# fallenshock/SinDDM

Measured on AMD Instinct MI355X. Metric: diffusion steps/sec (finest scale) + imgs/sec full multi-scale sample, 1/2/4/8 GPU, higher is better.
Workload: dtype f32 (3x3 convs: binary16 hi/lo split products -- Winograd-domain GEMMs with all 4 MFMA terms, fp32 accumulate; fp32-equivalent, error vs float64 = the fp32 oracle's: tests/test_gpu_h2.py; everything else fp32); 1 GPU; C3: 6-scale pyramid, T=1000, finest scale 411x512, batch 64 per GPU, dim=160; batch_per_gpu=64, global_batch=64, scale=5, parallelism=independent chains over 1 GPU(s), one all-gather of the images

## Files before the change

### include/sinddm_hip_debug.h

```cpp
#ifndef SINDDM_HIP_DEBUG_H
#define SINDDM_HIP_DEBUG_H

#include <stddef.h>
#include <stdint.h>

#ifdef __cplusplus
extern "C" {
#endif

int sinddm_prof_begin(void);
int sinddm_prof_end(double* conv_ms_total, int64_t* conv_launches, double* conv_flops_total);
int sinddm_prof_end2(double* conv_ms_total, int64_t* conv_launches, double* conv_flops_total,
                     double* conv_exec_flops_total);
int sinddm_prof_end3(int kind, double* ms_total, int64_t* launches, double* flops_total,
                     double* exec_flops_total, int reset);

int sinddm_debug_conv_path(int dim, int B, int H, int W);

int sinddm_debug_infer_path(int dim, int B, int H, int W);

int sinddm_debug_head_path(int dim, int B, int H, int W);
int sinddm_debug_head_offsets(int dim, int64_t out[3]);
int sinddm_debug_head(const float* packed, const float* g, const float* x_in, float* eps_out, int dim, int B, int H, int W,
                      int Wp, void* stream);

int sinddm_debug_train_path(int dim, int B, int H, int W);

int sinddm_debug_block_train(const float* params, const float* packed, const float* packed_bwd, int dim, int l,
                             const float* x, const float* cond_bias, const float* grad_y, float* y, float* grad_x,
                             float* grad_params, float* dcond, int B, int H, int W, void* ws, size_t ws_bytes,
                             void* stream);

int sinddm_debug_wgrad_map(int Cin, int Cout, int64_t ntiles, int ncu, uint32_t* wg_out, int wg_cap, int32_t* splits_out,
                           int splits_cap);

#ifdef __cplusplus
}
#endif
#endif
```

### sinddm_amd/_lib.py

```python
from __future__ import annotations

import ctypes as C
import os
from typing import Optional

import torch

_HERE = os.path.dirname(os.path.abspath(__file__))
LIB_PATH = os.path.join(_HERE, "libsinddm_hip.so")

ABI_SYMBOLS = (
    "sinddm_abi_version", "sinddm_param_count", "sinddm_param_tensors", "sinddm_param_offset",
    "sinddm_packed_count", "sinddm_workspace_bytes", "sinddm_pack_weights", "sinddm_net_forward",
    "sinddm_q_sample", "sinddm_reverse_step", "sinddm_reverse_step_edit", "sinddm_upsample_bilinear", "sinddm_prof_begin", "sinddm_prof_end", "sinddm_prof_end2", "sinddm_prof_end3", "sinddm_debug_wgrad_map", "sinddm_debug_conv_path",
    "sinddm_debug_block_train", "sinddm_debug_infer_path", "sinddm_debug_train_path",
    "sinddm_train_workspace_bytes", "sinddm_packed_bwd_count", "sinddm_pack_weights_bwd",
    "sinddm_net_forward_train", "sinddm_net_backward", "sinddm_l1_loss_fwd_bwd", "sinddm_adam_ema_step",
    "sinddm_cond_embed", "sinddm_cond_stride", "sinddm_sample_chain", "sinddm_sample_chain2", "sinddm_sample_chain_ex",
    "sinddm_normal_fill", "sinddm_wrap_halo", "sinddm_upsample_bilinear_wrap", "sinddm_sample_chain_tile",
    "sinddm_sample_chain_keep", "sinddm_reverse_step_keep", "sinddm_normal_fill_samples", "sinddm_sample_chain_seeds",
    "sinddm_debug_head_path", "sinddm_debug_head_offsets", "sinddm_debug_head",
)


ABI_VERSION = 3
DIM_FP32_CONVS = 0x10000
TILE_HALO = 16


class StepCoefs(C.Structure):
    _fields_ = [("mode", C.c_int), ("clip", C.c_int),
                ("sqrt_recip_ac_t", C.c_float), ("sqrt_recipm1_ac_t", C.c_float),
                ("coef1_t", C.c_float), ("coef2_t", C.c_float),
                ("gamma_t", C.c_float), ("gamma_tm1", C.c_float),
                ("sqrt_ac_tm1", C.c_float), ("sqrt_ac_t", C.c_float), ("sqrt_1m_ac_t", C.c_float),
                ("sqrt_1m_ac_tm1_mvar", C.c_float), ("sigma", C.c_float)]


class ChainOpts(C.Structure):
    _fields_ = [("edit_w", C.c_void_p), ("edit_c", C.c_void_p), ("noise", C.c_void_p)]


class KeepOpts(C.Structure):
    _fields_ = [("mask", C.c_void_p), ("x0", C.c_void_p), ("ab", C.POINTER(C.c_float))]


class SinddmError(RuntimeError):
    pass


_lib: Optional[C.CDLL] = None


def load() -> C.CDLL:
    global _lib
    if _lib is not None:
        return _lib
    if not os.path.exists(LIB_PATH):
        raise SinddmError(
# ... 17 lines not shown
        "sinddm_workspace_bytes": (sz, [i, i, i, i]),
        "sinddm_pack_weights": (i, [p, p, i, p]),
        "sinddm_net_forward": (i, [p, p, p, p, i, f, p, i, i, i, i, p, sz, p]),
        "sinddm_cond_embed": (i, [p, p, i, f, i, i, p, p, p, p]),
        "sinddm_cond_stride": (i, [i]),
        "sinddm_q_sample": (i, [p, p, p, p, p, p, p, p, i, i, i64, p]),
        "sinddm_reverse_step": (i, [p, p, p, p, p, C.POINTER(StepCoefs), i64, p]),
        "sinddm_reverse_step_edit": (i, [p, p, p, p, p, C.POINTER(StepCoefs), p, p, i, i, i, p]),
        "sinddm_sample_chain": (i, chain[:-2] + [C.POINTER(C.c_int)]),
        "sinddm_sample_chain2": (i, chain),
        "sinddm_sample_chain_ex": (i, chain + [C.POINTER(ChainOpts)]),
        "sinddm_sample_chain_tile": (i, chain + [C.POINTER(ChainOpts), i, i]),
        "sinddm_sample_chain_keep": (i, chain + [C.POINTER(ChainOpts), i, i, C.POINTER(KeepOpts)]),
        "sinddm_sample_chain_seeds": (i, chain + [C.POINTER(ChainOpts), i, i, C.POINTER(KeepOpts), p]),
        "sinddm_normal_fill_samples": (i, [p, i, i64, p, C.c_uint64, p]),
        "sinddm_reverse_step_keep": (i, [p, p, p, p, p, C.POINTER(StepCoefs), p, p, p, p, f, f, i, i, i, p]),
        "sinddm_wrap_halo": (i, [p, p, i, i, i, i, i, p]),
        "sinddm_upsample_bilinear_wrap": (i, [p, p, i, i, i, i, i, i, i, p]),
        "sinddm_normal_fill": (i, [p, i64, C.c_uint64, C.c_uint64, p]),
        "sinddm_upsample_bilinear": (i, [p, p, i, i, i, i, i, p]),
        "sinddm_prof_begin": (i, []),
        "sinddm_prof_end": (i, [C.POINTER(C.c_double), C.POINTER(C.c_int64), C.POINTER(C.c_double)]),
        "sinddm_prof_end2": (i, [C.POINTER(C.c_double), C.POINTER(C.c_int64), C.POINTER(C.c_double),
                                 C.POINTER(C.c_double)]),
        "sinddm_prof_end3": (i, [i, C.POINTER(C.c_double), C.POINTER(C.c_int64), C.POINTER(C.c_double),
                                 C.POINTER(C.c_double), i]),
        "sinddm_debug_wgrad_map": (i, [i, i, i64, i, C.POINTER(C.c_uint32), i, C.POINTER(C.c_int32), i]),
        "sinddm_debug_conv_path": (i, [i, i, i, i]),
        "sinddm_debug_infer_path": (i, [i, i, i, i]),
        "sinddm_debug_train_path": (i, [i, i, i, i]),
        "sinddm_debug_head_path": (i, [i, i, i, i]),
        "sinddm_debug_head_offsets": (i, [i, C.POINTER(C.c_int64)]),
        "sinddm_debug_head": (i, [p, p, p, p, i, i, i, i, i, p]),
        "sinddm_debug_block_train": (i, [p, p, p, i, i, p, p, p, p, p, p, p, i, i, i, p, sz, p]),
        "sinddm_train_workspace_bytes": (sz, [i, i, i, i]),
        "sinddm_packed_bwd_count": (i64, [i]),
        "sinddm_pack_weights_bwd": (i, [p, p, i, p]),
        "sinddm_net_forward_train": (i, [p, p, p, p, i, f, p, i, i, i, i, p, sz, p]),
        "sinddm_net_backward": (i, [p, p, p, p, p, p, p, i, i, i, i, p, sz, p]),
        "sinddm_l1_loss_fwd_bwd": (i, [p, p, p, p, i64, f, p]),
        "sinddm_adam_ema_step": (i, [p, p, p, p, p, f, f, f, f, f, f, f, i, i64, p]),
    }
    for name, (res, args) in sig.items():
        if not hasattr(lib, name):
            continue
        fn = getattr(lib, name)
        fn.restype = res
        fn.argtypes = args
    _lib = lib
    return lib


def missing_symbols():
    lib = load()
    return [s for s in ABI_SYMBOLS if not hasattr(lib, s)]


def check(rc: int, what: str) -> None:
    if rc != 0:
        kind = {-1: "bad argument", -2: "unsupported shape", -3: "workspace too small"}.get(rc, f"hipError {rc}")
        raise SinddmError(f"{what} failed: {kind}")


def ptr(t: Optional[torch.Tensor]) -> Optional[int]:
    if t is None:
        return None
# ... 10 lines not shown
```

### sinddm_amd/csrc/head.h

```cpp
#pragma once
#include "common.h"

namespace sinddm {

#ifndef SINDDM_HEAD_COLLAPSE
#define SINDDM_HEAD_COLLAPSE 1
#endif

constexpr int HEAD_GROUP = 16;

struct HeadPackArgs {
    long long dst;
    long long c2_w, c2_b, res_w, res_b;
    long long fin_w, fin_b;
    int half, dim;
};
__global__ __launch_bounds__(256) void head_pack_kernel(const float* __restrict__ params, float* __restrict__ packed,
                                                        HeadPackArgs a) {
    const int nc = a.half * CHANNELS * 9, nr = a.dim * CHANNELS;
    const int i = blockIdx.x * 256 + threadIdx.x;
    if (i >= nc + nr + CHANNELS) return;
    const float* wf = params + a.fin_w;
    double s = 0.;
    if (i < nc) {
        const int tap = i % 9, o = (i / 9) % CHANNELS, ci = i / (9 * CHANNELS);
        for (int m = 0; m < a.half; ++m)
            s += (double)wf[o * a.half + m] * (double)params[a.c2_w + ((long long)m * a.half + ci) * 9 + tap];
    } else if (i < nc + nr) {
        const int j = i - nc, o = j % CHANNELS, ci = j / CHANNELS;
        for (int m = 0; m < a.half; ++m) s += (double)wf[o * a.half + m] * (double)params[a.res_w + (long long)m * a.dim + ci];
    } else {
        const int o = i - nc - nr;
        for (int m = 0; m < a.half; ++m)
            s += (double)wf[o * a.half + m] * ((double)params[a.c2_b + m] + (double)params[a.res_b + m]);
        s += (double)params[a.fin_b + o];
    }
    packed[a.dst + i] = (float)s;
}

inline int head_pack_launch(const NetPlan& P, const float* params, float* packed, hipStream_t st) {
    const BlockPlan& b = P.blk[3];
    HeadPackArgs a{};
    a.dst = P.pk_hc;
    a.c2_w = b.c2_w; a.c2_b = b.c2_b; a.res_w = b.res_w; a.res_b = b.res_b;
    a.fin_w = P.fin_w; a.fin_b = P.fin_b;
    a.half = P.half; a.dim = P.dim;
    const long long total = P.npacked - P.pk_hc;
    hipLaunchKernelGGL(head_pack_kernel, dim3((unsigned)((total + 255) / 256)), dim3(256), 0, st, params, packed, a);
    SINDDM_LAUNCH_CHECK();
    return 0;
}

struct HeadEps {
    const float* g;
    const float* xin;
    const float* wc;
    const float* wr;
    const float* bc;
    int half, dim, H, Wp;

    __device__ __forceinline__ void operator()(int b, int q, f32x4 (&e)[3]) const {
        const int qpr = Wp >> 2;
        const int y = q / qpr, x = (q - y * qpr) * 4;
        const int plane = H * Wp;
        constexpr int OOBI = 0x40000000;
        int oq[3], ol[3], orr[3];
#pragma unroll
        for (int r = 0; r < 3; ++r) {
            const int gy = y + r - 1;
            const bool ok = gy >= 0 && gy < H;
            const int base = (gy * Wp + x) * 4;
            oq[r] = ok ? base : OOBI;
            ol[r] = (ok && x >= 4) ? base - 4 : OOBI;
            orr[r] = (ok && x + 4 < Wp) ? base + 16 : OOBI;
        }
#pragma unroll
        for (int o = 0; o < 3; ++o) e[o] = f32x4{bc[o], bc[o], bc[o], bc[o]};
        const float* gb = g + (size_t)b * half * plane;
        auto fetch = [&](int c, float (&v)[3][6]) __attribute__((always_inline)) {
            const __amdgpu_buffer_rsrc_t rs =
                __builtin_amdgcn_make_buffer_rsrc(const_cast<float*>(gb + (size_t)c * plane), 0, plane * 4, 0x00020000);
#pragma unroll
            for (int r = 0; r < 3; ++r) {
                const f32x4 m = __builtin_bit_cast(f32x4, __builtin_amdgcn_raw_buffer_load_b128(rs, oq[r], 0, 0));
                v[r][0] = __builtin_bit_cast(float, __builtin_amdgcn_raw_buffer_load_b32(rs, ol[r], 0, 0));
                v[r][1] = m[0]; v[r][2] = m[1]; v[r][3] = m[2]; v[r][4] = m[3];
                v[r][5] = __builtin_bit_cast(float, __builtin_amdgcn_raw_buffer_load_b32(rs, orr[r], 0, 0));
            }
        };
        float in[3][6];
        fetch(0, in);
        f32x4 p[3] = {{0.f, 0.f, 0.f, 0.f}, {0.f, 0.f, 0.f, 0.f}, {0.f, 0.f, 0.f, 0.f}};
        for (int c = 0; c < half; ++c) {
            float nx[3][6];
            fetch(c + 1 < half ? c + 1 : c, nx);
            const float* wk = wc + c * 27;
#pragma unroll
            for (int r = 0; r < 3; ++r)
#pragma unroll
                for (int o = 0; o < 3; ++o)
#pragma unroll
                    for (int kx = 0; kx < 3; ++kx)
#pragma unroll
                        for (int j = 0; j < 4; ++j) p[o][j] = fmaf(wk[o * 9 + r * 3 + kx], in[r][j + kx], p[o][j]);
            if ((c + 1) % HEAD_GROUP == 0 || c + 1 == half) {
#pragma unroll
                for (int o = 0; o < 3; ++o) {
                    e[o] += p[o];
                    p[o] = f32x4{0.f, 0.f, 0.f, 0.f};
                }
            }
#pragma unroll
            for (int r = 0; r < 3; ++r)
#pragma unroll
                for (int k = 0; k < 6; ++k) in[r][k] = nx[r][k];
        }
        const float* xb = xin + (size_t)b * dim * plane + (size_t)q * 4;
        for (int c0 = 0; c0 < dim; c0 += HEAD_GROUP) {
            const int c1 = c0 + HEAD_GROUP < dim ? c0 + HEAD_GROUP : dim;
            f32x4 p[3] = {{0.f, 0.f, 0.f, 0.f}, {0.f, 0.f, 0.f, 0.f}, {0.f, 0.f, 0.f, 0.f}};
#pragma unroll 8
            for (int c = c0; c < c1; ++c) {
                const f32x4 v = *reinterpret_cast<const f32x4*>(xb + (size_t)c * plane);
#pragma unroll
                for (int o = 0; o < 3; ++o)
#pragma unroll
                    for (int j = 0; j < 4; ++j) p[o][j] = fmaf(wr[c * 3 + o], v[j], p[o][j]);
            }
#pragma unroll
            for (int o = 0; o < 3; ++o) e[o] += p[o];
        }
    }
};

struct FinalConvEps {
    const float* a;
    const float* w;
    const float* bias;
    int C;
    size_t plane;

    __device__ __forceinline__ void operator()(int b, int q, f32x4 (&e)[3]) const {
        const float* src = a + (size_t)b * C * plane + (size_t)q * 4;
#pragma unroll
        for (int o = 0; o < 3; ++o) e[o] = f32x4{bias[o], bias[o], bias[o], bias[o]};
#pragma unroll 8
        for (int c = 0; c < C; ++c) {
            const f32x4 v = *reinterpret_cast<const f32x4*>(src + (size_t)c * plane);
// ... 34 lines not shown
```

### sinddm_amd/csrc/internal.h

```cpp
#pragma once
#include "common.h"

namespace sinddm {

struct PackSeg {
    long long dst;
    long long count;
    long long w;
    long long w2;
    int kind;
    int cin, cout, taps, nch, mt, co_lds;
    int transpose;
};
struct PackArgs {
    PackSeg seg[32];
    int nseg;
    long long total;
};
int pack_launch(const float* params, float* packed, const PackArgs& a, hipStream_t st);

struct TrainBufs {
    float* cond;
    float* emb;
    float* hpre;
    float* cvec;
    float* mvec;
    float* h[4];
    float* u[4];
    float* g[4];
    float* o[4];
    float* s[4];
    float* dcond;
    float* small;
    float* wscr;
    float* amax;
};

struct ChainStep;
int net_forward_impl(const NetPlan& P, const float* params, const float* packed, const float* x, const int64_t* t_dev,
                     int t_host, float scale, float* out, int B, int H, int W, void* ws, size_t ws_bytes,
                     hipStream_t st, const TrainBufs* tb, const ChainStep* cs = nullptr);

int block_forward(const NetPlan& P, int l, const float* params, const float* packed, const float* cur, const float* cond,
                  int cond_stride, float* hbuf, float* gbuf, float* obuf, float* upre, int B, int H, int W, hipStream_t st,
                  int Wt = 0, float* amax = nullptr, bool skip2 = false);
int conv3x3_path(int cout, int cin, int coblks, int B, int H, int W);

struct ConvArgs;
bool wh_applies(const NetPlan& P, int B, int H, int W, int cin, int cout);
bool wh_enabled();
int wh_conv(const ConvArgs& c, hipStream_t st);
int wh_pack(const float* w, float* wsinv, void* img, int cin, int cout, int transpose, hipStream_t st);
int amax_tensor_launch(const float* x, float* amax, int B, long long per_sample, hipStream_t st);

int dwconv_launch(const float* x, const float* w, const float* bias, const float* cond, int cond_stride,
                  const float* addt, int flip, float* out, int B, int C, int H, int W, hipStream_t st, int pi = 0, int po = 0,
                  float* amax = nullptr);

}
```

### sinddm_amd/csrc/plan.h

```cpp
#pragma once
#include <stdint.h>

namespace sinddm {

constexpr int KC = 8;
constexpr int TIME_DIM = 32;
constexpr int CHANNELS = 3;

inline bool wh_plan_ok(int cin, int cout) { return cin >= 32 && cin % 16 == 0 && cout % 80 == 0; }
inline long long wh_plan_halfs(int cin, int cout) { return (long long)(cout / 80) * (cin / 16) * 24 * 5 * 512; }

struct BlockPlan {
    int cin, cout;
    int64_t mlp_w, mlp_b, tr_w, tr_b, dw_w, dw_b, c1_w, c1_b, c2_w, c2_b, res_w, res_b;
    int mt;
    int coblks;
    int co_lds;
    int nch1;
    int nch2;
    int nchr;
    int64_t pk_c1, pk_c2, pk_res, pk_b1, pk_b2;
    int nchw1, nchw2;
    int64_t pk_wc1, pk_wc2;
    int64_t pk_w1f, pk_w2f;
    int64_t pk_q1, pk_q2, pk_qs1, pk_qs2;
    int cond_off;
};

struct NetPlan {
    int dim, half;
    BlockPlan blk[4];
    int64_t tm0_w, tm0_b, tm2_w, tm2_b, fin_w, fin_b;
    int64_t nparams, npacked;
    int64_t pk_zero;
    int64_t pk_hc, pk_hr, pk_hb;
    int ntensors;
    int64_t tensor_off[64];
    int cond_stride;
    bool fp32_convs;
    bool ok;
};

inline int mt_for(int cout) { return (cout % 80 == 0) ? 5 : ((cout % 32 == 0) ? 2 : 1); }
inline int co_lds_for(int mt) { int m = mt * 16; return (m % 32 == 16) ? m : m + 16; }

inline NetPlan make_plan(int dim_arg) {
    NetPlan p{};
    const int dim = dim_arg & 0xFFFF;
    p.fp32_convs = (dim_arg & 0x10000) != 0;
    if (dim_arg < 0 || (dim_arg >> 17) != 0) { p.ok = false; return p; }
    p.ok = dim >= 2 && dim % 2 == 0 && dim <= 1024;
    p.dim = dim;
    p.half = dim / 2;
    int64_t o = 0;
    int nt = 0;
    auto take = [&](int64_t n) { int64_t r = o; p.tensor_off[nt++] = r; o += n; return r; };
    p.tm0_w = take(TIME_DIM * 4 * TIME_DIM * 2);
    p.tm0_b = take(TIME_DIM * 4);
    p.tm2_w = take(TIME_DIM * TIME_DIM * 4);
    p.tm2_b = take(TIME_DIM);
    const int cins[4] = {CHANNELS, p.half, dim, dim};
    const int couts[4] = {p.half, dim, dim, p.half};
    int64_t q = 0;
    int coff = 0;
    for (int l = 0; l < 4; ++l) {
        BlockPlan& b = p.blk[l];
        b.cin = cins[l];
        b.cout = couts[l];
        b.mlp_w = take(TIME_DIM * TIME_DIM);
        b.mlp_b = take(TIME_DIM);
        b.tr_w = take((int64_t)b.cin * TIME_DIM);
        b.tr_b = take(b.cin);
        b.dw_w = take((int64_t)b.cin * 25);
        b.dw_b = take(b.cin);
        b.c1_w = take((int64_t)b.cout * b.cin * 9);
        b.c1_b = take(b.cout);
        b.c2_w = take((int64_t)b.cout * b.cout * 9);
        b.c2_b = take(b.cout);
        if (b.cin != b.cout) {
            b.res_w = take((int64_t)b.cout * b.cin);
            b.res_b = take(b.cout);
        } else {
            b.res_w = b.res_b = -1;
// ... 47 lines not shown
```

### sinddm_amd/csrc/sinddm_fwd.hip

```cpp
#include "conv_mfma.h"
#include "conv_wino.h"
#include "conv_wino4.h"
#include "conv_wh.h"
#include "internal.h"
#include "step_tail.h"
#include <type_traits>
namespace sinddm {

ConvProfiler& conv_profiler() {
    static ConvProfiler p;
    return p;
}

__global__ void pack_kernel(const float* __restrict__ params, float* __restrict__ packed, PackArgs a) {
    long long i = (long long)blockIdx.x * blockDim.x + threadIdx.x;
    if (i >= a.total) return;
    int s = 0;
    long long base = 0;
    while (s < a.nseg - 1 && i >= base + a.seg[s].count) { base += a.seg[s].count; ++s; }
    const PackSeg& g = a.seg[s];
    const long long j = i - base;
    float v = 0.0f;
    if (g.kind == 0) {
        const int co_l = (int)(j % g.co_lds);
// ... 414 lines not shown
        const f32x4 qr = __builtin_bit_cast(f32x4, __builtin_amdgcn_raw_buffer_load_b128(rsx, (rowok && rok) ? base + 16 : OOBI, 0, 0));
        const float in[8] = {ql[2], ql[3], qm[0], qm[1], qm[2], qm[3], qr[0], qr[1]};
#pragma unroll
        for (int r = 0; r < DWR_ROWS; ++r) {
            const int ky = ir - r;
            if (ky >= 0 && ky < 5) {
#pragma unroll
                for (int kx = 0; kx < 5; ++kx) {
#pragma unroll
                    for (int cc = 0; cc < 4; ++cc) acc[r][cc] = fmaf(wk[ky * 5 + kx], in[cc + kx], acc[r][cc]);
                }
            }
        }
    }
    float mx = 0.f;
#pragma unroll
    for (int r = 0; r < DWR_ROWS; ++r) {
        const int gy = y0 + r;
        if (colok && gy < H) {
            const size_t o = plane + (size_t)gy * W + x4;
            f32x4 v = acc[r];
            if (addt) v += *reinterpret_cast<const f32x4*>(addt + o);
            if (x4 + 4 > Wt) {
#pragma unroll
                for (int cc = 0; cc < 4; ++cc) v[cc] = x4 + cc < Wt ? v[cc] : 0.0f;
            }
            mx = fmaxf(fmaxf(mx, fmaxf(fabsf(v[0]), fabsf(v[1]))), fmaxf(fabsf(v[2]), fabsf(v[3])));
            *reinterpret_cast<f32x4*>(out + o) = v;
        }
    }
    if (amax) amax_publish(mx, amax + (size_t)b * AMAX_STRIDE);
}

#ifndef SINDDM_DW_ROWS
#define SINDDM_DW_ROWS 1
#endif

int dwconv_launch(const float* x, const float* w, const float* bias, const float* cond, int cond_stride,
                  const float* addt, int flip, float* out, int B, int C, int H, int W, hipStream_t st, int pi, int po,
                  float* amax) {
    if (pi <= 0) pi = W;
    if (po <= 0) po = W;
    if (SINDDM_DW_ROWS && pi % 4 == 0 && po == pi && pi >= 192) {
        const int bandsX = (pi + 255) / 256, bandsY = (H + 4 * DWR_ROWS - 1) / (4 * DWR_ROWS);
        hipLaunchKernelGGL(dwconv5_rows_kernel, dim3(bandsX * bandsY, C, B), dim3(256), 0, st, x, w, bias, cond, cond_stride,
                           addt, flip, out, C, H, pi, bandsX, W, amax);
        SINDDM_LAUNCH_CHECK();
        return 0;
    }
    const int tilesX = (W + DW_TW - 1) / DW_TW, tilesY = (H + DW_TH - 1) / DW_TH;
    const int groupsX = (tilesX + DW_NX - 1) / DW_NX;
    hipLaunchKernelGGL(dwconv5_kernel, dim3(groupsX * tilesY, C, B), dim3(256), 0, st, x, w, bias, cond, cond_stride,
                       addt, flip, out, C, H, W, groupsX, pi, po, amax);
    SINDDM_LAUNCH_CHECK();
    return 0;
}

__global__ __launch_bounds__(256) void conv3x3_c3_gelu_kernel(const float* __restrict__ in, const float* __restrict__ w,
                                                              const float* __restrict__ bias, float* __restrict__ out,
                                                              float* __restrict__ out_pre, int H, int W, int Cout,
                                                              int co_per_block, int Wt, float* __restrict__ amax) {
    const int HW = H * W;
    const int b = blockIdx.y;
    const int co0 = blockIdx.z * co_per_block;
    const int co1 = min(Cout, co0 + co_per_block);
    const int p = blockIdx.x * 256 + threadIdx.x;
    const bool live = p < HW;
    const int pc = live ? p : HW - 1;
    const int y = pc / W, x = pc - y * W;
    const float* src = in + (size_t)b * 3 * HW;
    float v[27];
#pragma unroll
    for (int ci = 0; ci < 3; ++ci)
#pragma unroll
        for (int ky = 0; ky < 3; ++ky)
#pragma unroll
            for (int kx = 0; kx < 3; ++kx) {
                const int gy = y + ky - 1, gx = x + kx - 1;
                const bool ok = gy >= 0 && gy < H && gx >= 0 && gx < W;
                v[ci * 9 + ky * 3 + kx] = ok ? src[(size_t)ci * HW + (size_t)gy * W + gx] : 0.0f;
            }
    float* dst = out + (size_t)b * Cout * HW + pc;
    float* dpre = out_pre ? out_pre + (size_t)b * Cout * HW + pc : nullptr;
    f32x2 vp[13];
#pragma unroll
    for (int j = 0; j < 13; ++j) vp[j] = f32x2{v[2 * j], v[2 * j + 1]};
// ... 250 lines not shown
        if (b.cin != 3 && !(b.pk_wc1 >= 0 && b.cin % 4 == 0)) return false;
    }
    return true;
}
static int fwd_pitch(const NetPlan& P, int W) { return (W % 4 != 0 && plan_pads_rows(P)) ? (W + 3) / 4 * 4 : W; }
static size_t fwd_xpad_bytes(const NetPlan& P, int B, int H, int W) {
    return fwd_pitch(P, W) != W ? align_up((size_t)B * CHANNELS * H * fwd_pitch(P, W) * sizeof(float), 256) : 0;
}
static size_t fwd_workspace_core(const NetPlan& P, int B, int H, int W) {
    const size_t act = align_up((size_t)B * P.dim * H * fwd_pitch(P, W) * sizeof(float), 256);
    return cond_region_bytes(P, B) + 4 * act + fwd_xpad_bytes(P, B, H, W);
}
static size_t fwd_workspace_bytes(const NetPlan& P, int B, int H, int W) {
    return fwd_workspace_core(P, B, H, W) + 2 * cond_region_bytes(P, (B + 1) / 2) + 4096;
}

struct ChainStep {
    const float* cond_row;
    const float* x_tilde;
    float* x_next;
    TailArgs tail;
};

template <class F>
static void tail_dispatch(const TailArgs& t, F&& f) {
    auto keep = [&](auto e, auto n) { t.km ? f(e, n, std::true_type{}) : f(e, n, std::false_type{}); };
    auto noise = [&](auto e) { t.nz ? keep(e, std::true_type{}) : keep(e, std::false_type{}); };
    t.ew ? noise(std::true_type{}) : noise(std::false_type{});
}

static bool head_applies(const TrainBufs* tb, int H, int Wp) {
    return SINDDM_HEAD_COLLAPSE && !tb && Wp % 4 == 0 && (long long)H * Wp < (1LL << 28);
}
static HeadEps head_eps(const NetPlan& P, const float* packed, const float* g, const float* xin, int H, int Wp) {
    return HeadEps{g, xin, packed + P.pk_hc, packed + P.pk_hr, packed + P.pk_hb, P.half, P.dim, H, Wp};
}

int conv3x3_path(int cout, int cin, int coblks, int B, int H, int W) {
    if (!wino_enabled() || cout % 4 != 0) return 0;
    const bool f24 = mt_for(cout) == 5 && cout % 80 == 0 && cin >= 16 && cin % 16 == 0;
    const bool v3 = SINDDM_WINO_V3 && f24 &&
                    (long long)B * ((W + 31) / 32) * ((H + 3) / 4) * coblks >= SINDDM_V3_MIN_ITEMS_PER_CU * wino2_cu_count();
    if (v3 && SINDDM_WINO_V4 && conv_wino4_applies(B, H, W, coblks)) return 4;
    return v3 ? 3 : 2;
}

int block_forward(const NetPlan& P, int l, const float* params, const float* packed, const float* cur, const float* cond,
                  int cond_stride, float* hbuf, float* gbuf, float* obuf, float* upre, int B, int H, int W, hipStream_t st,
                  int Wt, float* amax, bool skip2) {
    const BlockPlan& b = P.blk[l];
    const bool wha = amax && b.pk_q1 >= 0 && conv_wh_applies(P.fp32_convs, B, H, W, b.cin, b.cout);
    const bool whb = !skip2 && amax && b.pk_q2 >= 0 && conv_wh_applies(P.fp32_convs, B, H, W, b.cout, b.cout);
    int rc = Wt > 0 ? dwconv_launch(cur, params + b.dw_w, params + b.dw_b, cond, cond_stride, nullptr, 0, hbuf, B, b.cin, H,
                                    Wt, st, W, W, wha ? amax : nullptr)
                    : dwconv_launch(cur, params + b.dw_w, params + b.dw_b, cond, cond_stride, nullptr, 0, hbuf, B, b.cin, H,
                                    W, st, 0, 0, wha ? amax : nullptr);
    if (rc) return rc;
    const bool wino = wino_enabled();
    ConvArgs c1{};
    c1.in = hbuf; c1.bias = packed + b.pk_b1; c1.out = gbuf;
    c1.B = B; c1.H = H; c1.W = W; c1.Cin = b.cin; c1.Cout = b.cout; c1.nch1 = 0;
    c1.coblks = b.coblks; c1.act = 1; c1.zero = packed + P.pk_zero; c1.Wt = Wt;
    c1.out_pre = upre;
    constexpr int c3 = SINDDM_CONV_C3;
    const bool v3 = SINDDM_WINO_V3 && wino &&
                    (long long)B * ((W + 31) / 32) * ((H + 3) / 4) * b.coblks >= SINDDM_V3_MIN_ITEMS_PER_CU * wino2_cu_count();
    const bool v4 = SINDDM_WINO_V4 && v3 && conv_wino4_applies(B, H, W, b.coblks);
    if (wha) {
        c1.w3 = packed + b.pk_q1; c1.wsinv = packed + b.pk_qs1; c1.amax_in = amax; c1.amax_out = whb ? amax + 1 : nullptr;
        c1.bias = params + b.c1_b;
        rc = conv_wh_launch(c1, st);
    } else if (v3 && b.pk_w1f >= 0) {
        c1.w3 = packed + b.pk_w1f; c1.nch3 = b.nchw1;
        rc = v4 ? conv_wino4_launch(c1, st) : conv_wino3_launch(c1, st);
    } else if (wino && b.pk_wc1 >= 0 && b.cin % 4 == 0) {
        c1.w3 = packed + b.pk_wc1; c1.nch3 = b.nchw1;
        rc = conv_wino_launch(c1, b.mt, st);
    } else if (b.cin == 3 && c3) {
        const int nwg = ((H * W + 255) / 256) * B;
        int split = 1;
        while (split < 8 && nwg * split < 2048 && b.cout % (split * 2) == 0) split *= 2;
        hipLaunchKernelGGL(conv3x3_c3_gelu_kernel, dim3((H * W + 255) / 256, B, split), dim3(256), 0, st, hbuf,
                           params + b.c1_w, params + b.c1_b, gbuf, c1.out_pre, H, W, b.cout, b.cout / split, Wt > 0 ? Wt : W,
                           whb ? amax + 1 : nullptr);
        SINDDM_LAUNCH_CHECK();
        rc = 0;
// ... 97 lines not shown

    CondArgs ca = cond_args(P, params);
    ca.t_dev = reinterpret_cast<const long long*>(t_dev); ca.t_host = t_host; ca.scale = scale;
    ca.out = fb.cond;
    ca.cond_vec = tb ? tb->cvec : nullptr; ca.hidden = tb ? tb->hpre : nullptr;
    ca.emb_out = tb ? tb->emb : nullptr; ca.mvec_out = tb ? tb->mvec : nullptr;
    if (!cs) {
        hipLaunchKernelGGL(cond_kernel, dim3(B), dim3(128), 0, st, ca);
        SINDDM_LAUNCH_CHECK();
    }

    const bool head = head_applies(tb, H, Wp);
    if (amax) {
        bool any = false;
        for (int l = 0; l < 4; ++l) {
            const BlockPlan& b = P.blk[l];
            any = any || (b.pk_q1 >= 0 && conv_wh_applies(P.fp32_convs, B, H, Wp, b.cin, b.cout)) ||
                  (!(head && l == 3) && b.pk_q2 >= 0 && conv_wh_applies(P.fp32_convs, B, H, Wp, b.cout, b.cout));
        }
        if (!any) amax = nullptr;
        else if (hipMemsetAsync(amax, 0, (size_t)B * AMAX_STRIDE * sizeof(float), st) != hipSuccess) return SINDDM_E_BADARG;
    }
    const float* cur = x;
    if (padded) {
        const long long nrows = (long long)B * CHANNELS * H;
        const long long nq = nrows * (Wp / 4);
        hipLaunchKernelGGL(pad_rows_kernel, dim3((unsigned)((nq + 255) / 256)), dim3(256), 0, st, x, xpad, H, W, Wp, nrows);
        SINDDM_LAUNCH_CHECK();
        cur = xpad;
    }
    int freeb[4] = {0, 1, 2, 3};
    int curb = -1;
    const float* head_g = nullptr;
    for (int l = 0; l < 4; ++l) {
        const BlockPlan& b = P.blk[l];
        int sel[3], n = 0;
        for (int i = 0; i < 4 && n < 3; ++i)
            if (freeb[i] != curb) sel[n++] = freeb[i];
        float* hbuf = tb ? tb->h[l] : fb.buf[sel[0]];
        float* gbuf = tb ? tb->g[l] : fb.buf[sel[1]];
        float* obuf = tb ? tb->o[l] : fb.buf[sel[2]];
        const bool skip2 = head && l == 3;
        const int rc = block_forward(P, l, params, packed, cur, fb.cond + b.cond_off, cond_stride, hbuf, gbuf, obuf,
                                     tb ? tb->u[l] : nullptr, B, H, Wp, st, padded ? W : 0, amax ? amax + 2 * l : nullptr,
                                     skip2);
        if (rc) return rc;
        if (skip2) { head_g = gbuf; break; }
        cur = obuf;
        curb = sel[2];
    }
    const int HW = H * W;
    if (head) {
        const HeadEps he = head_eps(P, packed, head_g, cur, H, Wp);
        const dim3 grid((unsigned)((H * (Wp / 4) + 255) / 256), B);
        if (cs && cs->x_next && padded)
            tail_dispatch(cs->tail, [&](auto E, auto N, auto K) {
                hipLaunchKernelGGL((final_conv_reverse_step_pitch_kernel<decltype(E)::value, decltype(N)::value, decltype(K)::value, HeadEps>),
                                   grid, dim3(256), 0, st, he, x, cs->x_tilde, cs->x_next, H, W, Wp, cs->tail);
            });
        else if (cs && cs->x_next)
            tail_dispatch(cs->tail, [&](auto E, auto N, auto K) {
                hipLaunchKernelGGL((final_conv_reverse_step_kernel<decltype(E)::value, decltype(N)::value, decltype(K)::value, HeadEps>),
                                   grid, dim3(256), 0, st, he, x, cs->x_tilde, cs->x_next, HW, cs->tail);
            });
        else
            hipLaunchKernelGGL(head_eps_kernel, grid, dim3(256), 0, st, he, out, W);
        SINDDM_LAUNCH_CHECK();
        return 0;
    }
    const FinalConvEps fe{cur, params + P.fin_w, params + P.fin_b, P.half, (size_t)H * Wp};
    if (padded) {
        const unsigned gx = (unsigned)((H * (Wp / 4) + 255) / 256);
        if (cs && cs->x_next)
            tail_dispatch(cs->tail, [&](auto E, auto N, auto K) {
                hipLaunchKernelGGL((final_conv_reverse_step_pitch_kernel<decltype(E)::value, decltype(N)::value, decltype(K)::value, FinalConvEps>),
                                   dim3(gx, B), dim3(256), 0, st, fe, x, cs->x_tilde, cs->x_next, H, W, Wp, cs->tail);
            });
        else
            hipLaunchKernelGGL(final_conv1x1_pitch_kernel, dim3(gx, B), dim3(256), 0, st, cur, params + P.fin_w,
                               params + P.fin_b, out, P.half, H, W, Wp);
        SINDDM_LAUNCH_CHECK();
        return 0;
    }
    if (cs && cs->x_next && HW % 4 == 0) {
        tail_dispatch(cs->tail, [&](auto E, auto N, auto K) {
            hipLaunchKernelGGL((final_conv_reverse_step_kernel<decltype(E)::value, decltype(N)::value, decltype(K)::value, FinalConvEps>),
// ... 403 lines not shown
                     double* conv_exec_flops_total) {
    return sinddm_prof_end3(0, conv_ms_total, conv_launches, conv_flops_total, conv_exec_flops_total, 1);
}

int sinddm_debug_infer_path(int dim, int B, int H, int W) {
    NetPlan p = make_plan(dim);
    if (!p.ok || B <= 0 || H <= 0 || W <= 0) return SINDDM_E_BADARG;
    const BlockPlan& b = p.blk[2];
    const int Wp = fwd_pitch(p, W);
    if (b.pk_q2 >= 0 && conv_wh_applies(p.fp32_convs, B, H, Wp, b.cout, b.cout)) return 8;
    return conv3x3_path(b.cout, b.cout, b.coblks, B, H, Wp);
}

int sinddm_debug_head_path(int dim, int B, int H, int W) {
    NetPlan p = make_plan(dim);
    if (!p.ok || B <= 0 || H <= 0 || W <= 0) return SINDDM_E_BADARG;
    return head_applies(nullptr, H, fwd_pitch(p, W)) ? 1 : 0;
}

int sinddm_debug_head_offsets(int dim, int64_t out[3]) {
    NetPlan p = make_plan(dim);
    if (!p.ok || !out) return SINDDM_E_BADARG;
    out[0] = p.pk_hc; out[1] = p.pk_hr; out[2] = p.pk_hb;
    return 0;
}

int sinddm_debug_head(const float* packed, const float* g, const float* x_in, float* eps_out, int dim, int B, int H, int W,
                      int Wp, void* stream) {
    if (!packed || !g || !x_in || !eps_out || B <= 0 || H <= 0 || W <= 0) return SINDDM_E_BADARG;
    NetPlan p = make_plan(dim);
    if (!p.ok) return SINDDM_E_BADSHAPE;
    if (Wp % 4 != 0 || W > Wp || W <= Wp - 4 || (long long)H * Wp >= (1LL << 28) || B > 65535) return SINDDM_E_BADSHAPE;
    hipLaunchKernelGGL(head_eps_kernel, dim3((unsigned)((H * (Wp / 4) + 255) / 256), B), dim3(256), 0,
                       static_cast<hipStream_t>(stream), head_eps(p, packed, g, x_in, H, Wp), eps_out, W);
    SINDDM_LAUNCH_CHECK();
    return 0;
}

int sinddm_prof_end3(int kind, double* ms_total, int64_t* launches, double* flops_total, double* exec_flops_total,
                     int reset) {
    ConvProfiler& p = conv_profiler();
    p.on = false;
    double ms = 0.0, fl = 0.0, ex = 0.0;
    int64_t n = 0;
    for (int i = 0; i < p.used; ++i) {
        if (kind >= 10 ? (p.kind[i] != kind / 10 || p.gen[i] != kind % 10) : (kind != 0 && p.kind[i] != kind)) continue;
        hipError_t e = hipEventSynchronize(p.ev[2 * i + 1]);
        if (e != hipSuccess) return (int)e;
        float t = 0.f;
        e = hipEventElapsedTime(&t, p.ev[2 * i], p.ev[2 * i + 1]);
        if (e != hipSuccess) return (int)e;
        ms += t; fl += p.rec_flops[i]; ex += p.rec_exec[i]; ++n;
    }
    if (ms_total) *ms_total = ms;
    if (launches) *launches = n;
    if (flops_total) *flops_total = fl;
    if (exec_flops_total) *exec_flops_total = ex;
    if (reset) { p.used = 0; p.flops = 0.0; p.exec_flops = 0.0; }
    return 0;
}

int sinddm_upsample_bilinear(const float* in, float* out, int BC, int h, int w, int H, int W, void* stream) {
    if (!in || !out || BC <= 0 || h <= 0 || w <= 0 || H <= 0 || W <= 0) return SINDDM_E_BADARG;
    const float sy = (float)h / (float)H, sx = (float)w / (float)W;
    hipLaunchKernelGGL((upsample_bilinear_kernel<false, false>), dim3((H * W + 255) / 256, BC), dim3(256), 0,
                       static_cast<hipStream_t>(stream), in, out, h, w, H, W, sy, sx);
    SINDDM_LAUNCH_CHECK();
    return 0;
}
// ... 23 lines not shown
```

### sinddm_amd/models.py

```python
from __future__ import annotations

import ctypes as C
import math
from functools import partial
from pathlib import Path
from typing import Dict, Optional, Tuple

import numpy as np
import torch
import torch.nn.functional as F
from torch import nn

from . import _lib
from .functions import cosine_beta_schedule, default, exists, extract, noise_like
from .synth import net_param_shapes


class EMA:
    def __init__(self, beta):
        self.beta = beta

    def update_model_average(self, ma_model, current_model):
        for cur, ma in zip(current_model.parameters(), ma_model.parameters()):
            ma.data = self.update_average(ma.data, cur.data)
# ... 91 lines not shown

def _aux_stream(device: torch.device) -> int:
    device = torch.device(device)
    idx = device.index if device.index is not None else torch.cuda.current_device()
    st = _AUX.get(idx)
    if st is None:
        st = torch.cuda.Stream(device=idx)
        _AUX[idx] = st
    return st.cuda_stream


class _Leaf(nn.Module):

    def __init__(self, wshape, fan_in):
        super().__init__()
        w = torch.empty(wshape)
        nn.init.kaiming_uniform_(w, a=math.sqrt(5))
        bound = 1 / math.sqrt(fan_in) if fan_in > 0 else 0
        b = torch.empty(wshape[0]).uniform_(-bound, bound)
        self.weight = nn.Parameter(w)
        self.bias = nn.Parameter(b)


def _container(children: Dict[str, nn.Module]) -> nn.Module:
    m = nn.Module()
    for k, v in children.items():
        m.add_module(k, v)
    return m


class SinDDMNet(nn.Module):

    fp32_convs = False

    def __init__(self, dim, out_dim=None, channels=3, with_time_emb=True, multiscale=False, device=None):
        super().__init__()
        if not with_time_emb or not multiscale:
            raise NotImplementedError("the MI355X build implements the configuration main.py uses: "
                                      "with_time_emb=True, multiscale=True (reference main.py:77-81); the reference's own forward "
                                      "cannot run any other combination (models.py:136-141)")
        if channels != 3 or default(out_dim, channels) != 3:
            raise NotImplementedError("channels=3 / out_dim=3 only (reference main.py:77-81, models.py:129)")
        self.device = device
        self.channels = channels
        self.multiscale = multiscale
        self.dim = int(dim)
        time_dim = 32
        half = int(dim / 2)
        self.SinEmbTime = SinusoidalPosEmb(time_dim)
        self.SinEmbScale = SinusoidalPosEmb(time_dim)
        self.time_mlp = _container({"0": _Leaf((time_dim * 4, time_dim * 2), time_dim * 2),
                                    "2": _Leaf((time_dim, time_dim * 4), time_dim * 4)})
        for name, (cin, cout) in zip(("l1", "l2", "l3", "l4"),
                                     ((channels, half), (half, dim), (dim, dim), (dim, half))):
            kids = {
                "mlp": _container({"1": _Leaf((time_dim, time_dim), time_dim)}),
                "time_reshape": _Leaf((cin, time_dim, 1, 1), time_dim),
                "ds_conv": _Leaf((cin, 1, 5, 5), 25),
                "net": _container({"0": _Leaf((cout, cin, 3, 3), cin * 9), "2": _Leaf((cout, cout, 3, 3), cout * 9)}),
            }
            if cin != cout:
                kids["res_conv"] = _Leaf((cout, cin, 1, 1), cin)
            self.add_module(name, _container(kids))
        self.final_conv = _container({"0": _Leaf((channels, half, 1, 1), half)})

        self._flat: Optional[torch.Tensor] = None
# ... 99 lines not shown
            if self._packed_bwd is None:
                self._packed_bwd = torch.empty(lib.sinddm_packed_bwd_count(self.dim), dtype=torch.float32,
                                               device=self._flat.device)
            _lib.check(lib.sinddm_pack_weights_bwd(_lib.ptr(self._flat), _lib.ptr(self._packed_bwd), self.dim,
                                                   _lib.stream_ptr(self._flat.device)), "sinddm_pack_weights_bwd")
            self._packed_bwd_version = v
        return self._packed_bwd

    def infer(self, x: torch.Tensor, t_dev: Optional[torch.Tensor], t_host: int, scale: float,
              out: Optional[torch.Tensor] = None) -> torch.Tensor:
        lib = _lib.load()
        if not x.is_cuda:
            raise _lib.SinddmError("SinDDMNet needs a ROCm device tensor: there is no CPU fallback")
        x = x.contiguous()
        if x.dtype != torch.float32:
            raise _lib.SinddmError("fp32 only")
        B, Cc, H, W = x.shape
        assert Cc == self.channels
        if out is None:
            out = torch.empty_like(x)
        packed = self.packed_weights()
        nbytes = lib.sinddm_workspace_bytes(self.dim, B, H, W)
        ws = _workspace(x.device, nbytes)
        if t_dev is not None:
            t_dev = t_dev.to(device=x.device, dtype=torch.int64).contiguous()
        _lib.check(lib.sinddm_net_forward(_lib.ptr(self._flat), _lib.ptr(packed), _lib.ptr(x),
                                          _lib.ptr(t_dev) if t_dev is not None else None, int(t_host),
                                          float(scale), _lib.ptr(out), self.dim_arg, B, H, W, ws.data_ptr(),
                                          ws.numel(), _lib.stream_ptr(x.device)), "sinddm_net_forward")
        return out

    @property
    def dim_arg(self) -> int:
        return self.dim | (_lib.DIM_FP32_CONVS if self.fp32_convs else 0)

    def forward(self, x, time, scale=None):
        s = float(scale) if scale is not None else 0.0
        needs_grad = torch.is_grad_enabled() and any(p.requires_grad for p in self.parameters())
        if needs_grad:
            from .autograd import net_forward_train
            return net_forward_train(self, x, time, s)
        return self.infer(x, time, 0, s)


class MultiScaleGaussianDiffusion(nn.Module):

    def __init__(self, denoise_fn, *, save_interm=False, results_folder='/Results', n_scales, scale_factor,
                 image_sizes, scale_mul=(1, 1), channels=3, timesteps=100, train_full_t=False, scale_losses=None,
                 loss_factor=1, loss_type='l1', betas=None, device=None, reblurring=True, sample_limited_t=False,
                 omega=0):
        super().__init__()
        self.device = device
        self.save_interm = save_interm
        self.results_folder = Path(results_folder)
        self.channels = channels
        self.n_scales = n_scales
        self.scale_factor = scale_factor
        self.scale_mul = scale_mul
        self.sample_limited_t = sample_limited_t
        self.reblurring = reblurring
        self.img_prev_upsample = None

        self.clip_guided_sampling = False
        self.guidance_sub_iters = None
        self.stop_guidance = None
        self.quantile = 0.8
        self.clip_model = None
# ... 657 lines not shown
```

Measured before the change: 759.9 sample-steps/s (finest scale, batch x steps/s, all GPUs).

## Fuse head residual 1x1 projection into last block's depthwise conv

Result: no change. 762.8 sample-steps/s (finest scale, batch x steps/s, all GPUs), median of 6 (+0.4%).

```diff
diff --git a/include/sinddm_hip_debug.h b/include/sinddm_hip_debug.h
--- a/include/sinddm_hip_debug.h
+++ b/include/sinddm_hip_debug.h
@@ -24,6 +24,11 @@
 int sinddm_debug_head(const float* packed, const float* g, const float* x_in, float* eps_out, int dim, int B, int H, int W,
                       int Wp, void* stream);
 
+#define SINDDM_DIM_DEBUG_NO_HEAD_PROJ 0x20000
+int sinddm_debug_head_proj_path(int dim, int B, int H, int W);
+int sinddm_debug_dw_proj(const float* params, const float* packed, const float* x_in, const float* cond_bias, float* h,
+                         float* part, float* amax, int dim, int B, int H, int W, int Wp, int proj, void* stream);
+
 int sinddm_debug_train_path(int dim, int B, int H, int W);
 
 int sinddm_debug_block_train(const float* params, const float* packed, const float* packed_bwd, int dim, int l,
diff --git a/sinddm_amd/_lib.py b/sinddm_amd/_lib.py
--- a/sinddm_amd/_lib.py
+++ b/sinddm_amd/_lib.py
@@ -20,11 +20,13 @@
     "sinddm_normal_fill", "sinddm_wrap_halo", "sinddm_upsample_bilinear_wrap", "sinddm_sample_chain_tile",
     "sinddm_sample_chain_keep", "sinddm_reverse_step_keep", "sinddm_normal_fill_samples", "sinddm_sample_chain_seeds",
     "sinddm_debug_head_path", "sinddm_debug_head_offsets", "sinddm_debug_head",
+    "sinddm_debug_head_proj_path", "sinddm_debug_dw_proj",
 )
 
 
 ABI_VERSION = 3
 DIM_FP32_CONVS = 0x10000
+DIM_DEBUG_NO_HEAD_PROJ = 0x20000
 TILE_HALO = 16
 
 
@@ -108,6 +110,8 @@
         "sinddm_debug_head_path": (i, [i, i, i, i]),
         "sinddm_debug_head_offsets": (i, [i, C.POINTER(C.c_int64)]),
         "sinddm_debug_head": (i, [p, p, p, p, i, i, i, i, i, p]),
+        "sinddm_debug_head_proj_path": (i, [i, i, i, i]),
+        "sinddm_debug_dw_proj": (i, [p, p, p, p, p, p, p, i, i, i, i, i, i, p]),
         "sinddm_debug_block_train": (i, [p, p, p, i, i, p, p, p, p, p, p, p, i, i, i, p, sz, p]),
         "sinddm_train_workspace_bytes": (sz, [i, i, i, i]),
         "sinddm_packed_bwd_count": (i64, [i]),
diff --git a/sinddm_amd/csrc/head.h b/sinddm_amd/csrc/head.h
--- a/sinddm_amd/csrc/head.h
+++ b/sinddm_amd/csrc/head.h
@@ -54,6 +54,7 @@
 struct HeadEps {
     const float* g;
     const float* xin;
+    const float* part;
     const float* wc;
     const float* wr;
     const float* bc;
@@ -114,6 +115,19 @@
             for (int r = 0; r < 3; ++r)
 #pragma unroll
                 for (int k = 0; k < 6; ++k) in[r][k] = nx[r][k];
+        }
+        if (part) {
+            const int ng = dim / HEAD_GROUP;
+            const float* pb = part + (size_t)b * ng * CHANNELS * plane + (size_t)q * 4;
+#pragma unroll 2
+            for (int gi = 0; gi < ng; ++gi) {
+                f32x4 p[3];
+#pragma unroll
+                for (int o = 0; o < 3; ++o) p[o] = *reinterpret_cast<const f32x4*>(pb + (size_t)(gi * CHANNELS + o) * plane);
+#pragma unroll
+                for (int o = 0; o < 3; ++o) e[o] += p[o];
+            }
+            return;
         }
         const float* xb = xin + (size_t)b * dim * plane + (size_t)q * 4;
         for (int c0 = 0; c0 < dim; c0 += HEAD_GROUP) {
diff --git a/sinddm_amd/csrc/internal.h b/sinddm_amd/csrc/internal.h
--- a/sinddm_amd/csrc/internal.h
+++ b/sinddm_amd/csrc/internal.h
@@ -43,7 +43,7 @@
 
 int block_forward(const NetPlan& P, int l, const float* params, const float* packed, const float* cur, const float* cond,
                   int cond_stride, float* hbuf, float* gbuf, float* obuf, float* upre, int B, int H, int W, hipStream_t st,
-                  int Wt = 0, float* amax = nullptr, bool skip2 = false);
+                  int Wt = 0, float* amax = nullptr, bool skip2 = false, float* head_part = nullptr);
 int conv3x3_path(int cout, int cin, int coblks, int B, int H, int W);
 
 struct ConvArgs;
diff --git a/sinddm_amd/csrc/plan.h b/sinddm_amd/csrc/plan.h
--- a/sinddm_amd/csrc/plan.h
+++ b/sinddm_amd/csrc/plan.h
@@ -38,6 +38,7 @@
     int64_t tensor_off[64];
     int cond_stride;
     bool fp32_convs;
+    bool no_head_proj;
     bool ok;
 };
 
@@ -48,7 +49,8 @@
     NetPlan p{};
     const int dim = dim_arg & 0xFFFF;
     p.fp32_convs = (dim_arg & 0x10000) != 0;
-    if (dim_arg < 0 || (dim_arg >> 17) != 0) { p.ok = false; return p; }
+    p.no_head_proj = (dim_arg & 0x20000) != 0;
+    if (dim_arg < 0 || (dim_arg >> 18) != 0) { p.ok = false; return p; }
     p.ok = dim >= 2 && dim % 2 == 0 && dim <= 1024;
     p.dim = dim;
     p.half = dim / 2;
diff --git a/sinddm_amd/csrc/sinddm_fwd.hip b/sinddm_amd/csrc/sinddm_fwd.hip
--- a/sinddm_amd/csrc/sinddm_fwd.hip
+++ b/sinddm_amd/csrc/sinddm_fwd.hip
@@ -470,6 +470,104 @@
     if (amax) amax_publish(mx, amax + (size_t)b * AMAX_STRIDE);
 }
 
+#ifndef DWP_ROWS_
+#define DWP_ROWS_ 4
+#endif
+constexpr int DWP_ROWS = DWP_ROWS_;
+static_assert(DWP_ROWS >= 1 && DWP_ROWS <= 12, "DWP_ROWS");
+
+__global__ __launch_bounds__(256) void dwconv5_rows_proj_kernel(const float* __restrict__ x, const float* __restrict__ w,
+                                                                 const float* __restrict__ bias, const float* __restrict__ cond,
+                                                                 int cond_stride, const float* __restrict__ wr,
+                                                                 float* __restrict__ out, float* __restrict__ part, int C,
+                                                                 int H, int W, int bandsX, int Wt, float* __restrict__ amax) {
+    const int grp = blockIdx.y, b = blockIdx.z;
+    const int by = blockIdx.x / bandsX, bx = blockIdx.x - by * bandsX;
+    const int lane = threadIdx.x & 63, wv = threadIdx.x >> 6;
+    const int x4 = (bx * 64 + lane) * 4;
+    const int y0 = (by * 4 + wv) * DWP_ROWS;
+    if (y0 >= H) return;
+    constexpr int OOBI = 0x40000000;
+    const bool colok = x4 < W;
+    const bool lok = colok && x4 >= 4, rok = colok && x4 + 4 < W;
+    f32x4 p[DWP_ROWS][CHANNELS];
+#pragma unroll
+    for (int r = 0; r < DWP_ROWS; ++r)
+#pragma unroll
+        for (int o = 0; o < CHANNELS; ++o) p[r][o] = f32x4{0.f, 0.f, 0.f, 0.f};
+    float mx = 0.f;
+#pragma unroll 1
+    for (int c = grp * HEAD_GROUP; c < (grp + 1) * HEAD_GROUP; ++c) {
+        const size_t plane = ((size_t)b * C + c) * H * W;
+        float wk[25];
+#pragma unroll
+        for (int k = 0; k < 25; ++k) wk[k] = w[c * 25 + k];
+        const float wo[CHANNELS] = {wr[c * CHANNELS], wr[c * CHANNELS + 1], wr[c * CHANNELS + 2]};
+        const float add = (bias ? bias[c] : 0.0f) + (cond ? cond[(size_t)b * cond_stride + c] : 0.0f);
+        const __amdgpu_buffer_rsrc_t rsx = __builtin_amdgcn_make_buffer_rsrc(const_cast<float*>(x + plane), 0, H * W * 4, 0x00020000);
+        f32x4 acc[DWP_ROWS];
+#pragma unroll
+        for (int r = 0; r < DWP_ROWS; ++r) acc[r] = f32x4{add, add, add, add};
+#pragma unroll
+        for (int ir = 0; ir < DWP_ROWS + 4; ++ir) {
+            const int gy = y0 + ir - 2;
+            const bool rowok = gy >= 0 && gy < H;
+            const int base = (gy * W + x4) * 4;
+            const f32x4 ql = __builtin_bit_cast(f32x4, __builtin_amdgcn_raw_buffer_load_b128(rsx, (rowok && lok) ? base - 16 : OOBI, 0, 0));
+            const f32x4 qm = __builtin_bit_cast(f32x4, __builtin_amdgcn_raw_buffer_load_b128(rsx, (rowok && colok) ? base : OOBI, 0, 0));
+            const f32x4 qr = __builtin_bit_cast(f32x4, __builtin_amdgcn_raw_buffer_load_b128(rsx, (rowok && rok) ? base + 16 : OOBI, 0, 0));
+            const float in[8] = {ql[2], ql[3], qm[0], qm[1], qm[2], qm[3], qr[0], qr[1]};
+            if (ir >= 2 && ir < DWP_ROWS + 2) {
+#pragma unroll
+                for (int o = 0; o < CHANNELS; ++o)
+#pragma unroll
+                    for (int cc = 0; cc < 4; ++cc) p[ir - 2][o][cc] = fmaf(wo[o], qm[cc], p[ir - 2][o][cc]);
+            }
+#pragma unroll
+            for (int r = 0; r < DWP_ROWS; ++r) {
+                const int ky = ir - r;
+                if (ky >= 0 && ky < 5) {
+#pragma unroll
+                    for (int kx = 0; kx < 5; ++kx) {
+#pragma unroll
+                        for (int cc = 0; cc < 4; ++cc) acc[r][cc] = fmaf(wk[ky * 5 + kx], in[cc + kx], acc[r][cc]);
+                    }
+                }
+            }
+        }
+#pragma unroll
+        for (int r = 0; r < DWP_ROWS; ++r) {
+            const int gy = y0 + r;
+            if (colok && gy < H) {
+                f32x4 v = acc[r];
+                if (x4 + 4 > Wt) {
+#pragma unroll
+                    for (int cc = 0; cc < 4; ++cc) v[cc] = x4 + cc < Wt ? v[cc] : 0.0f;
+                }
+                mx = fmaxf(fmaxf(mx, fmaxf(fabsf(v[0]), fabsf(v[1]))), fmaxf(fabsf(v[2]), fabsf(v[3])));
+                *reinterpret_cast<f32x4*>(out + plane + (size_t)gy * W + x4) = v;
+            }
+        }
+    }
+    const size_t part0 = ((size_t)b * gridDim.y + grp) * CHANNELS * H * W;
+#pragma unroll
+    for (int r = 0; r < DWP_ROWS; ++r) {
+        const int gy = y0 + r;
+        if (colok && gy < H) {
+#pragma unroll
+            for (int o = 0; o < CHANNELS; ++o) {
+                f32x4 v = p[r][o];
+                if (x4 + 4 > Wt) {
+#pragma unroll
+                    for (int cc = 0; cc < 4; ++cc) v[cc] = x4 + cc < Wt ? v[cc] : 0.0f;
+                }
+                *reinterpret_cast<f32x4*>(part + part0 + ((size_t)o * H + gy) * W + x4) = v;
+            }
+        }
+    }
+    if (amax) amax_publish(mx, amax + (size_t)b * AMAX_STRIDE);
+}
+
 #ifndef SINDDM_DW_ROWS
 #define SINDDM_DW_ROWS 1
 #endif
@@ -490,6 +588,25 @@
     const int groupsX = (tilesX + DW_NX - 1) / DW_NX;
     hipLaunchKernelGGL(dwconv5_kernel, dim3(groupsX * tilesY, C, B), dim3(256), 0, st, x, w, bias, cond, cond_stride,
                        addt, flip, out, C, H, W, groupsX, pi, po, amax);
+    SINDDM_LAUNCH_CHECK();
+    return 0;
+}
+
+#ifndef SINDDM_HEAD_PROJ_IN_DW
+#define SINDDM_HEAD_PROJ_IN_DW 1
+#endif
+
+static bool dw_proj_applies(const NetPlan& P, int pitch) {
+    return SINDDM_HEAD_PROJ_IN_DW && SINDDM_DW_ROWS && !P.no_head_proj && P.dim % HEAD_GROUP == 0 && pitch % 4 == 0 &&
+           pitch >= 192;
+}
+
+static int dwconv_proj_launch(const float* x, const float* w, const float* bias, const float* cond, int cond_stride,
+                              const float* wr, float* out, float* part, int B, int C, int H, int W, hipStream_t st, int pitch,
+                              float* amax) {
+    const int bandsX = (pitch + 255) / 256, bandsY = (H + 4 * DWP_ROWS - 1) / (4 * DWP_ROWS);
+    hipLaunchKernelGGL(dwconv5_rows_proj_kernel, dim3(bandsX * bandsY, C / HEAD_GROUP, B), dim3(256), 0, st, x, w, bias, cond,
+                       cond_stride, wr, out, part, C, H, pitch, bandsX, W, amax);
     SINDDM_LAUNCH_CHECK();
     return 0;
 }
@@ -806,8 +923,9 @@
 static bool head_applies(const TrainBufs* tb, int H, int Wp) {
     return SINDDM_HEAD_COLLAPSE && !tb && Wp % 4 == 0 && (long long)H * Wp < (1LL << 28);
 }
-static HeadEps head_eps(const NetPlan& P, const float* packed, const float* g, const float* xin, int H, int Wp) {
-    return HeadEps{g, xin, packed + P.pk_hc, packed + P.pk_hr, packed + P.pk_hb, P.half, P.dim, H, Wp};
+static HeadEps head_eps(const NetPlan& P, const float* packed, const float* g, const float* xin, const float* part, int H,
+                        int Wp) {
+    return HeadEps{g, xin, part, packed + P.pk_hc, packed + P.pk_hr, packed + P.pk_hb, P.half, P.dim, H, Wp};
 }
 
 int conv3x3_path(int cout, int cin, int coblks, int B, int H, int W) {
@@ -821,11 +939,13 @@
 
 int block_forward(const NetPlan& P, int l, const float* params, const float* packed, const float* cur, const float* cond,
                   int cond_stride, float* hbuf, float* gbuf, float* obuf, float* upre, int B, int H, int W, hipStream_t st,
-                  int Wt, float* amax, bool skip2) {
+                  int Wt, float* amax, bool skip2, float* head_part) {
     const BlockPlan& b = P.blk[l];
     const bool wha = amax && b.pk_q1 >= 0 && conv_wh_applies(P.fp32_convs, B, H, W, b.cin, b.cout);
     const bool whb = !skip2 && amax && b.pk_q2 >= 0 && conv_wh_applies(P.fp32_convs, B, H, W, b.cout, b.cout);
-    int rc = Wt > 0 ? dwconv_launch(cur, params + b.dw_w, params + b.dw_b, cond, cond_stride, nullptr, 0, hbuf, B, b.cin, H,
+    int rc = head_part ? dwconv_proj_launch(cur, params + b.dw_w, params + b.dw_b, cond, cond_stride, packed + P.pk_hr, hbuf,
+                                            head_part, B, b.cin, H, Wt > 0 ? Wt : W, st, W, wha ? amax : nullptr)
+             : Wt > 0 ? dwconv_launch(cur, params + b.dw_w, params + b.dw_b, cond, cond_stride, nullptr, 0, hbuf, B, b.cin, H,
                                     Wt, st, W, W, wha ? amax : nullptr)
                     : dwconv_launch(cur, params + b.dw_w, params + b.dw_b, cond, cond_stride, nullptr, 0, hbuf, B, b.cin, H,
                                     W, st, 0, 0, wha ? amax : nullptr);
@@ -989,6 +1109,7 @@
     int freeb[4] = {0, 1, 2, 3};
     int curb = -1;
     const float* head_g = nullptr;
+    const float* head_part = nullptr;
     for (int l = 0; l < 4; ++l) {
         const BlockPlan& b = P.blk[l];
         int sel[3], n = 0;
@@ -1000,15 +1121,19 @@
         const bool skip2 = head && l == 3;
         const int rc = block_forward(P, l, params, packed, cur, fb.cond + b.cond_off, cond_stride, hbuf, gbuf, obuf,
                                      tb ? tb->u[l] : nullptr, B, H, Wp, st, padded ? W : 0, amax ? amax + 2 * l : nullptr,
-                                     skip2);
+                                     skip2, skip2 && dw_proj_applies(P, Wp) ? obuf : nullptr);
         if (rc) return rc;
-        if (skip2) { head_g = gbuf; break; }
+        if (skip2) {
+            head_g = gbuf;
+            if (dw_proj_applies(P, Wp)) head_part = obuf;
+            break;
+        }
         cur = obuf;
         curb = sel[2];
     }
     const int HW = H * W;
     if (head) {
-        const HeadEps he = head_eps(P, packed, head_g, cur, H, Wp);
+        const HeadEps he = head_eps(P, packed, head_g, cur, head_part, H, Wp);
         const dim3 grid((unsigned)((H * (Wp / 4) + 255) / 256), B);
         if (cs && cs->x_next && padded)
             tail_dispatch(cs->tail, [&](auto E, auto N, auto K) {
@@ -1478,9 +1603,32 @@
     if (!p.ok) return SINDDM_E_BADSHAPE;
     if (Wp % 4 != 0 || W > Wp || W <= Wp - 4 || (long long)H * Wp >= (1LL << 28) || B > 65535) return SINDDM_E_BADSHAPE;
     hipLaunchKernelGGL(head_eps_kernel, dim3((unsigned)((H * (Wp / 4) + 255) / 256), B), dim3(256), 0,
-                       static_cast<hipStream_t>(stream), head_eps(p, packed, g, x_in, H, Wp), eps_out, W);
+                       static_cast<hipStream_t>(stream), head_eps(p, packed, g, x_in, nullptr, H, Wp), eps_out, W);
     SINDDM_LAUNCH_CHECK();
     return 0;
+}
+
+int sinddm_debug_head_proj_path(int dim, int B, int H, int W) {
+    NetPlan p = make_plan(dim);
+    if (!p.ok || B <= 0 || H <= 0 || W <= 0) return SINDDM_E_BADARG;
+    const int Wp = fwd_pitch(p, W);
+    return head_applies(nullptr, H, Wp) && dw_proj_applies(p, Wp) ? 1 : 0;
+}
+
+int sinddm_debug_dw_proj(const float* params, const float* packed, const float* x_in, const float* cond_bias, float* h,
+                         float* part, float* amax, int dim, int B, int H, int W, int Wp, int proj, void* stream) {
+    if (!params || !packed || !x_in || !cond_bias || !h || !amax || (proj && !part) || B <= 0 || H <= 0 || W <= 0)
+        return SINDDM_E_BADARG;
+    NetPlan p = make_plan(dim);
+    if (!p.ok) return SINDDM_E_BADSHAPE;
+    if (Wp % 4 != 0 || W > Wp || W <= Wp - 4 || (long long)H * Wp >= (1LL << 28) || B > 65535) return SINDDM_E_BADSHAPE;
+    if (proj && !dw_proj_applies(p, Wp)) return SINDDM_E_BADSHAPE;
+    const BlockPlan& b = p.blk[3];
+    hipStream_t st = static_cast<hipStream_t>(stream);
+    if (proj)
+        return dwconv_proj_launch(x_in, params + b.dw_w, params + b.dw_b, cond_bias, b.cin, packed + p.pk_hr, h, part, B, b.cin,
+                                  H, W, st, Wp, amax);
+    return dwconv_launch(x_in, params + b.dw_w, params + b.dw_b, cond_bias, b.cin, nullptr, 0, h, B, b.cin, H, W, st, Wp, Wp, amax);
 }
 
 int sinddm_prof_end3(int kind, double* ms_total, int64_t* launches, double* flops_total, double* exec_flops_total,
diff --git a/sinddm_amd/models.py b/sinddm_amd/models.py
--- a/sinddm_amd/models.py
+++ b/sinddm_amd/models.py
@@ -147,6 +147,7 @@
 class SinDDMNet(nn.Module):
 
     fp32_convs = False
+    head_proj = True
 
     def __init__(self, dim, out_dim=None, channels=3, with_time_emb=True, multiscale=False, device=None):
         super().__init__()
@@ -312,7 +313,7 @@
 
     @property
     def dim_arg(self) -> int:
-        return self.dim | (_lib.DIM_FP32_CONVS if self.fp32_convs else 0)
+        return self.dim | (_lib.DIM_FP32_CONVS if self.fp32_convs else 0) | (0 if self.head_proj else _lib.DIM_DEBUG_NO_HEAD_PROJ)
 
     def forward(self, x, time, scale=None):
         s = float(scale) if scale is not None else 0.0
```
